# davidea97/Fisher-Nerf-customized

Hardware: AMD Instinct MI355X
Metric: candidate-views/sec (higher is better)
Workload: dtype f32

## Files before the change

### fisher-nerf-customized_amd/csrc/fisher_rast.hip

```cpp
#include <hip/hip_runtime.h>
#include <hip/hip_fp16.h>
#include <stdint.h>
#include <stdio.h>
#include <stdlib.h>
#include <string.h>
#include "fr_math.h"
#include "fr_sortnet.h"
#include "../../include/fisher_rast.h"
#include "fr_internal.h"

#define FR_THREADS 256
#define FR_G_MAX 32
#define FR_MAX_LDS_TILES 4096
#define FR_PART_MIN_DEFAULT 2048
#define FR_SORT_SMALL_KEYS 2048
#define FR_SORT_MID_KEYS 4096
#define FR_SORT_BIG_KEYS 16384
#define FR_VC_MAX 16
#define FR_BATCH 256
#define FR_BWD_BATCH 128

#include <vector>
#include <utility>
static thread_local char g_err[512] = "";
// ... 6 lines not shown
#define FR_AB_ONLY(x) x
static int fr_debug_mode();
static int fr_env_int(const char* name) { const char* e = getenv(name); return e ? atoi(e) : 0; }
#else
#define FR_AB_ONLY(x)
static constexpr int fr_debug_mode() { return 0; }
#endif
static bool g_prof_on = false;
static std::vector<std::pair<hipEvent_t, hipEvent_t>> g_prof_events;
int fr_fail(int code, const char* msg)
{
	snprintf(g_err, sizeof(g_err), "%s", msg);
	return code;
}
int fr_check_launch(const char* what)
{
	hipError_t e = hipGetLastError();
	if (e != hipSuccess)
	{
		snprintf(g_err, sizeof(g_err), "%s: %s", what, hipGetErrorString(e));
		return FR_ELAUNCH;
	}
	return FR_OK;
}

struct FrSplat { float x, y, cx, cy, cz, o, depth; uint32_t ext; };

struct FrVisEntry { uint32_t idx, depth_bits, xy0, xy1; };

struct FrParams {
	int P, V, W, H;
	uint32_t gx, gy;
	int T;
	int G;
	float tanfovx, tanfovy, focal_x, focal_y, mod;
	int D, M;
	const float* bg; const float* view; const float* proj; const float* campos;
	const float* w2c;
	const float* means3D; const float* colors; const float* shs; const float* opac;
	const float* scales; const float* rots;
	const float* cov3D;
	float* cov3D_out;
	int* radii;
	FrSplat* splat;
	float* rgb;
	uint8_t* clamped;
	uint32_t* tile_cnt; uint32_t* tile_off; uint32_t* tile_fill;
	uint64_t* keys; long long key_capacity;
	uint32_t* blk_base;
	uint32_t* big_list;
	uint32_t* view_work;
	uint32_t* part_list;
	uint32_t* view_perm;
	int* status;
	int* vis_count;
	int* num_rendered;
	struct FrVisEntry* vis_list;
	uint32_t* vis_n;
	int VC;
	uint32_t tile_cap;
	uint32_t small_max;
	const uint32_t* order;
	int legacy_sort;
	int prefiltered;
	int ablate;
};
#ifdef FR_ABLATE
#define FR_ABL(x) x
#else
#define FR_ABL(x)
#endif

__device__ __forceinline__ float wave_sum(float v)
{
#pragma unroll
	for (int o = 32; o > 0; o >>= 1) v += __shfl_xor(v, o, 64);
	return v;
}
__device__ __forceinline__ int wave_max_i(int v)
{
#pragma unroll
	for (int o = 32; o > 0; o >>= 1) { int t = __shfl_xor(v, o, 64); v = t > v ? t : v; }
	return v;
}

__device__ __forceinline__ bool fr_any(bool x) { return __builtin_amdgcn_ballot_w64(x) != 0ull; }
__device__ __forceinline__ bool fr_all(bool x) { return __builtin_amdgcn_ballot_w64(!x) == 0ull; }
__device__ __forceinline__ float fr_readlane_f(float x, int l) { return __int_as_float(__builtin_amdgcn_readlane(__float_as_int(x), l)); }
__device__ __forceinline__ float fr_bperm_f(float x, int l) { return __int_as_float(__builtin_amdgcn_ds_bpermute(l << 2, __float_as_int(x))); }

__device__ __forceinline__ float fr_exp_hw(float x) { return __builtin_amdgcn_exp2f(x * 1.44269504088896341f); }

__device__ __forceinline__ float fr_power_threshold(float opacity)
{
	return (opacity > 0.f) ? (-__logf(255.0f * opacity) - 0.01f) : INFINITY;
}

__device__ __forceinline__ uint32_t fr_alpha_extent(float cx, float cy, float cz, float opacity)
{
	const float thr = fr_power_threshold(opacity);
	float hx = INFINITY, hy = INFINITY;
	if (!(thr <= 0.f)) { hx = -1.f; hy = -1.f; }
	else
	{
		const float det = cx * cz - cy * cy;
		if (det > 0.f && cx > 0.f && cz > 0.f)
// ... 70 lines not shown
		if (p.prefiltered && p_view.z <= 0.001f) p.status[3] = 1;
		if (!(p_view.z <= 0.001f))
		{
			float c3[6];
#pragma unroll
			for (int k = 0; k < 6; k++) c3[k] = p.cov3D[6 * (size_t)i + k];
			s = fr_preprocess_one(po, c3, vm, pm, p.W, p.H, p.tanfovx, p.tanfovy, p.focal_x, p.focal_y, p.gx, p.gy);
		}
		p.radii[vP + i] = s.radius;
		if (s.radius > 0)
		{
			nvis++;
			float4* dst = (float4*)(p.splat + vP + i);
			dst[0] = make_float4(s.px, s.py, s.conx, s.cony);
			dst[1] = make_float4(s.conz, p.opac[i], s.depth, __uint_as_float(fr_alpha_extent(s.conx, s.cony, s.conz, p.opac[i])));
			if (p.colors == nullptr)
			{
				fr_f3 cp = { p.campos[0], p.campos[1], p.campos[2] };
				uint8_t cl[3];
				fr_f3 c = fr_sh_to_rgb(p.D, po, cp, p.shs + 3 * (size_t)i * p.M, cl);
				p.rgb[3 * (vP + i)] = c.x; p.rgb[3 * (vP + i) + 1] = c.y; p.rgb[3 * (vP + i) + 2] = c.z;
				p.clamped[3 * (vP + i)] = cl[0]; p.clamped[3 * (vP + i) + 1] = cl[1]; p.clamped[3 * (vP + i) + 2] = cl[2];
			}
			for (uint32_t y = s.rect.y0; y < s.rect.y1; y++)
				for (uint32_t x = s.rect.x0; x < s.rect.x1; x++)
				{
					if (lds_hist) atomicAdd(&hist[y * p.gx + x], 1u);
					else atomicAdd(&cnt[y * p.gx + x], 1u);
				}
		}
	}
	if (lds_hist)
	{
		__syncthreads();
		for (int t = tid; t < p.T; t += FR_THREADS)
		{
			uint32_t c = hist[t];
			if (c)
			{
				const uint32_t before = atomicAdd(&cnt[t], c);
				if (p.blk_base) p.blk_base[((size_t)v * gridDim.x + blockIdx.x) * p.T + t] = before;
			}
		}
	}
	if (p.vis_count)
	{
		int s = nvis;
#pragma unroll
		for (int o = 32; o > 0; o >>= 1) s += __shfl_xor(s, o, 64);
		if ((tid & 63) == 0 && s) atomicAdd(&p.vis_count[v], s);
	}
}

__device__ __forceinline__ void fr_deal_views(const uint32_t* __restrict__ work, uint32_t* __restrict__ perm, int V, int tid, int nthreads)
{
	__shared__ uint32_t s_work[1024];
	for (int v = tid; v < V; v += nthreads) s_work[v] = __hip_atomic_load(work + v, __ATOMIC_RELAXED, __HIP_MEMORY_SCOPE_AGENT);
	__syncthreads();
	for (int v = tid; v < V; v += nthreads)
	{
		const uint32_t w = s_work[v];
		int rank = 0;
		for (int u = 0; u < V; u++)
		{
			const uint32_t wu = s_work[u];
			rank += (wu > w || (wu == w && u < v)) ? 1 : 0;
		}
		const int r = rank >> 3, j = rank & 7;
		perm[r * 8 + ((r & 1) ? 7 - j : j)] = (uint32_t)v;
	}
}

__global__ __launch_bounds__(1024) void k_scan_tiles(const uint32_t* __restrict__ cnt, uint32_t* __restrict__ off,
                                                     uint32_t* __restrict__ fill, int N, int T, int V,
                                                     long long capacity, int* __restrict__ status,
                                                     int* __restrict__ num_rendered, uint32_t* __restrict__ big_list,
                                                     uint32_t* __restrict__ view_work, uint32_t* __restrict__ view_perm)
{
	__shared__ uint32_t wsum[16];
	__shared__ uint32_t chunk_total;
	const int tid = threadIdx.x, lane = tid & 63, wave = tid >> 6;
	uint32_t carry = 0, maxc = 0;
	constexpr int PER = 16;
	for (int sbase = 0; sbase < N; sbase += 1024 * PER)
	{
		const int i0 = sbase + tid * PER;
		uint32_t c[PER];
		uint32_t s = 0;
		const bool whole = i0 + PER <= N;
		if (whole)
		{
#pragma unroll
			for (int q = 0; q < PER / 4; q++)
			{
				const uint4 t4 = ((const uint4*)(cnt + i0))[q];
				c[4 * q] = t4.x; c[4 * q + 1] = t4.y; c[4 * q + 2] = t4.z; c[4 * q + 3] = t4.w;
			}
		}
		else
		{
#pragma unroll
			for (int q = 0; q < PER; q++) c[q] = (i0 + q < N) ? cnt[i0 + q] : 0u;
		}
#pragma unroll
		for (int q = 0; q < PER; q++)
		{
			s += c[q];
			maxc = c[q] > maxc ? c[q] : maxc;
			if (c[q] > (uint32_t)FR_SORT_SMALL_KEYS) big_list[16 + atomicAdd(&big_list[0], 1u)] = (uint32_t)(i0 + q);
		}
		uint32_t x = s;
#pragma unroll
		for (int d = 1; d < 64; d <<= 1)
		{
			uint32_t y = __shfl_up(x, d, 64);
			if (lane >= d) x += y;
		}
		if (lane == 63) wsum[wave] = x;
		__syncthreads();
		if (wave == 0)
		{
			uint32_t ws = lane < 16 ? wsum[lane] : 0u;
			uint32_t incl = ws;
// ... 862 lines not shown
#pragma unroll
			for (int b = 0; b < NB; b++)
			{
				const uint32_t e = e0 + b * FR_THREADS + tid;
				const uint32_t lo = ev[b] ? vend[ev[b] - 1] : 0u;
				const uint64_t key = ((uint64_t)en[b].x << 32) | ((blockIdx.x * cap + (e - lo)) << 4);
				const uint32_t r = en[b].y;
				const uint32_t x0 = r & 255u, s0 = (r >> 8) & 255u, x1 = x0 + ((r >> 16) & 255u), s1 = s0 + (r >> 24);
				const uint32_t* hb = hist + (size_t)ev[b] * p.T;
				uint32_t* cu = cursor + (size_t)ev[b] * p.T;
				if (x1 > x0 && s1 > s0)
				for (uint32_t y = s0 >> 2; y <= (s1 - 1u) >> 2; y++)
				{
					const uint32_t a = max(s0, 4u * y) - 4u * y, z = min(s1, 4u * y + 4u) - 4u * y;
					const uint64_t ky = key | (uint64_t)(((1u << z) - 1u) & ~((1u << a) - 1u));
					for (uint32_t x = x0; x < x1; x++)
					{
						const uint32_t t = y * p.gx + x;
						const uint32_t base = hb[t];
						const uint32_t k = atomicAdd(&cu[t], 1u);
						FR_ABL(if (p.ablate != 32 && p.ablate != 33))
						if (base != 0xffffffffu) p.keys[base + k] = ky;
					}
				}
			}
			if (more)
			{
#pragma unroll
				for (int b = 0; b < NB; b++) { en[b] = nx[b]; ev[b] = nxv[b]; }
			}
		}
	}
	else
	{
		for (int vv = 0; vv < nv; vv++)
		{
			const int v = v0 + vv;
			uint32_t* cnt = p.tile_cnt + (size_t)v * p.T;
			const uint32_t* h = hist + (size_t)vv * p.T;
			for (int t = tid; t < p.T; t += FR_THREADS)
			{
				const uint32_t c = h[t];
				if (c) p.blk_base[((size_t)v * nblk + blockIdx.x) * p.T + t] = atomicAdd(&cnt[t], c);
			}
		}
	}
	if (tid < nv)
	{
		const int v = v0 + tid;
		p.vis_n[(size_t)v * nblk + blockIdx.x] = s_n[tid];
		if (p.vis_count && s_n[tid]) atomicAdd(&p.vis_count[v], (int)s_n[tid]);
		if (p.num_rendered && s_ref[tid]) atomicAdd(&p.num_rendered[v], (int)s_ref[tid]);
	}
}
__global__ __launch_bounds__(FR_THREADS) void k_scatter_vis(FrParams p)
{
	extern __shared__ uint32_t fr_dyn_lds[];
	uint32_t* s_cnt = fr_dyn_lds;
	uint32_t* s_base = fr_dyn_lds + p.T;
	if (p.status[1]) return;
	const int tid = threadIdx.x;
	const int v = blockIdx.y;
	const uint32_t nblk = gridDim.x;
	const uint32_t n = p.vis_n[(size_t)v * nblk + blockIdx.x];
	if (n == 0) return;
	const uint32_t* off = p.tile_off + (size_t)v * p.T;
	const uint32_t* bb = p.blk_base + ((size_t)v * nblk + blockIdx.x) * p.T;
	for (int t = tid; t < p.T; t += FR_THREADS) { s_cnt[t] = 0; s_base[t] = off[t] + bb[t]; }
	__syncthreads();
	const uint4* list = (const uint4*)(p.vis_list + ((size_t)v * nblk + blockIdx.x) * (size_t)(FR_THREADS * p.G));
	constexpr int NB = 4;
	for (uint32_t e0 = 0; e0 < n; e0 += NB * FR_THREADS)
	{
		uint4 en[NB];
#pragma unroll
		for (int b = 0; b < NB; b++)
		{
			const uint32_t e = e0 + b * FR_THREADS + tid;
			en[b] = e < n ? list[e] : make_uint4(0u, 0u, 0u, 0u);
		}
#pragma unroll
		for (int b = 0; b < NB; b++)
		{
			const uint64_t key = ((uint64_t)en[b].y << 32) | en[b].x;
			const uint32_t x0 = en[b].z & 0xffffu, y0 = en[b].z >> 16, x1 = en[b].w & 0xffffu, y1 = en[b].w >> 16;
			for (uint32_t y = y0; y < y1; y++)
				for (uint32_t x = x0; x < x1; x++)
				{
					const uint32_t t = y * p.gx + x;
					p.keys[s_base[t] + atomicAdd(&s_cnt[t], 1u)] = key;
				}
		}
	}
}

__device__ __forceinline__ void fr_tile_of_block(const FrParams& p, uint32_t& tile, int& v, uint32_t first = 0u)
{
	const uint32_t L = blockIdx.x - first;
	if ((p.V & 7) == 0)
	{
		const uint32_t xcd = L & 7u, q = L >> 3;
		v = (int)((q / (uint32_t)p.T) * 8u + xcd);
		if (p.view_perm) v = (int)p.view_perm[v];
		tile = q % (uint32_t)p.T;
	}
	else
// ... 5190 lines not shown
	{
		if (hipDeviceGetAttribute(&cus, hipDeviceAttributeMultiprocessorCount, dev) != hipSuccess || cus <= 0) cus = 256;
		device = dev;
		(void)hipGetLastError();
	}
	return cus;
}

struct FrJoinGuard {
	hipStream_t s; FrSideStream* side[2] = { nullptr, nullptr }; int n = 0;
	explicit FrJoinGuard(hipStream_t caller) : s(caller) {}
	void forked(FrSideStream* ss) { side[n++] = ss; }
	int join()
	{
		int rc = FR_OK;
		for (int i = 0; i < n; i++)
		{
			if (hipEventRecord(side[i]->join, side[i]->stream) != hipSuccess || hipStreamWaitEvent(s, side[i]->join, 0) != hipSuccess)
				rc = fr_fail(FR_ELAUNCH, "side stream join failed");
		}
		n = 0;
		return rc;
	}
	~FrJoinGuard() { if (n) { char keep[sizeof(g_err)]; memcpy(keep, g_err, sizeof(keep)); (void)join(); memcpy(g_err, keep, sizeof(keep)); } }
};

enum class FrRecForm {
	Score,
	A,
	General,
	Pose,
	Render,
	Point,
};
struct FrScorerPlan {
	FrRecForm form = FrRecForm::Score;
	int columns;
	FrRecordArgs ra;
	bool skip_pack = false;
	bool view_identity = false;
};
template <int C> __global__ void k_pack_static(FrParams p, const float* __restrict__ H_inv, float* __restrict__ packed, float4* __restrict__ mt, float4* __restrict__ grp);
template <int C, bool LIST, bool FORM_A> __global__ void k_fisher_records(FrParams p, FrRecordArgs ra);

static int fr_bin_pipeline(FrParams& p, const fr_gaussians* g, hipStream_t s, const FrScorerPlan* plan = nullptr)
{
	int rc;
	const int P = p.P;
	{
		FrZeroer z;
		z.add(p.tile_cnt, (size_t)p.V * p.T * 4); z.add(p.status, 16); z.add(p.big_list, 64);
		if (p.part_list) z.add(p.part_list, 4);
		if (p.view_work) z.add(p.view_work, (size_t)p.V * 4);
		if (p.vis_count) z.add(p.vis_count, (size_t)p.V * 4);
		if (p.num_rendered && p.vis_list != nullptr && p.T <= FR_MAX_LDS_TILES) z.add(p.num_rendered, (size_t)p.V * 4);
		z.launch(s);
	}
	const bool multi = p.vis_list != nullptr && p.T <= FR_MAX_LDS_TILES;
	if (g->cov3D_precomp) p.cov3D = g->cov3D_precomp;
	else if (plan && multi) p.cov3D = nullptr;
	else
	{
		hipLaunchKernelGGL(k_cov3d, dim3((P + FR_THREADS - 1) / FR_THREADS), dim3(FR_THREADS), 0, s, P, g->scales, p.mod, g->rotations, p.cov3D_out);
		if ((rc = fr_check_launch("k_cov3d"))) return rc;
		p.cov3D = p.cov3D_out;
	}
	p.G = multi ? fr_pick_G_views(P) : fr_pick_G(P, p.V);
	p.VC = fr_pick_VC(p.T);
	const int per_block = FR_THREADS * p.G;
	dim3 gridP((P + per_block - 1) / per_block, p.V);
	const size_t hist_lds = p.T <= FR_MAX_LDS_TILES ? (size_t)p.T * 4 : 16;
	if (plan && !plan->skip_pack)
	{
		const float* shared_hinv = plan->ra.hinv_stride ? nullptr : plan->ra.H_inv;
		dim3 gp((P + FR_THREADS - 1) / FR_THREADS);
		if (plan->columns == 4) hipLaunchKernelGGL((k_pack_static<4>), gp, dim3(FR_THREADS), 0, s, p, shared_hinv, (float*)plan->ra.packed, (float4*)plan->ra.mt, (float4*)plan->ra.grp);
		else hipLaunchKernelGGL((k_pack_static<11>), gp, dim3(FR_THREADS), 0, s, p, shared_hinv, (float*)plan->ra.packed, (float4*)plan->ra.mt, (float4*)plan->ra.grp);
		if ((rc = fr_check_launch("k_pack_static"))) return rc;
	}
	FrJoinGuard joins(s);
	if (multi)
	{
		const bool once = plan && plan->ra.comp != nullptr && fr_debug_mode() != 20;
		if (!once) p.tile_cap = 0;
		const bool wanted_fixed = p.tile_cap != 0;
		if (once) p.VC = fr_plan_views_c(p.T, p.VC, p.tile_cap);
		if (once && wanted_fixed && !p.tile_cap) return fr_fail(FR_EINVAL, "fr_bin_pipeline: fixed key segments planned, but they do not fit the LDS");
		auto lds_c_of = [&](int vc) { return fr_lds_views_c(vc, p.T, p.tile_cap != 0); };
		dim3 gridV(gridP.x, (p.V + p.VC - 1) / p.VC);
		const size_t lds = ((size_t)p.VC * p.T + (size_t)FR_THREADS * p.VC + 12 * (size_t)p.VC + 2 * (size_t)p.VC * 8 * (size_t)p.G) * 4;
		FrRecordArgs ra = plan ? plan->ra : FrRecordArgs{ nullptr, 0, nullptr, nullptr, nullptr, nullptr, 0, nullptr, nullptr, 6 };
		const bool dk = p.tile_cap != 0;
		const size_t lds_c = lds_c_of(p.VC);
#define FR_VIEWS_C(...) hipLaunchKernelGGL((k_preprocess_views_c<__VA_ARGS__>), gridV, dim3(FR_THREADS), lds_c, s, p, ra)
		const bool c4 = plan && plan->columns == 4;
		if (once)
		{
			switch (plan->form)
			{
			case FrRecForm::Render:
				if (dk) FR_VIEWS_C(4, 4, true); else FR_VIEWS_C(4, 4, false);
				break;
			case FrRecForm::Pose:
				if (dk) FR_VIEWS_C(4, 3, true); else FR_VIEWS_C(4, 3, false);
				break;
			case FrRecForm::General:
				if (c4) { if (dk) FR_VIEWS_C(4, 2, true); else FR_VIEWS_C(4, 2, false); }
				else { if (dk) FR_VIEWS_C(11, 2, true); else FR_VIEWS_C(11, 2, false); }
				break;
			case FrRecForm::A:
				if (dk) FR_VIEWS_C(4, 1, true); else FR_VIEWS_C(4, 1, false);
				break;
			case FrRecForm::Point:
				if (c4) { if (dk) FR_VIEWS_C(4, 0, true, false, true); else FR_VIEWS_C(4, 0, false, false, true); }
				else { if (dk) FR_VIEWS_C(11, 0, true, false, true); else FR_VIEWS_C(11, 0, false, false, true); }
				break;
			case FrRecForm::Score:
				if (c4 && dk && plan->view_identity) FR_VIEWS_C(4, 0, true, true);
				else if (c4) { if (dk) FR_VIEWS_C(4, 0, true); else FR_VIEWS_C(4, 0, false); }
				else { if (dk) FR_VIEWS_C(11, 0, true); else FR_VIEWS_C(11, 0, false); }
				break;
			}
		}
#undef FR_VIEWS_C
		else if (!plan) hipLaunchKernelGGL((k_preprocess_views<0, false>), gridV, dim3(FR_THREADS), lds, s, p, ra);
#ifdef FR_AB
		else if (plan->form == FrRecForm::A) hipLaunchKernelGGL((k_preprocess_views<-4, true>), gridV, dim3(FR_THREADS), lds, s, p, ra);
		else if (c4) hipLaunchKernelGGL((k_preprocess_views<4, true>), gridV, dim3(FR_THREADS), lds, s, p, ra);
		else hipLaunchKernelGGL((k_preprocess_views<11, true>), gridV, dim3(FR_THREADS), lds, s, p, ra);
#else
		else return fr_fail(FR_EINVAL, "fr_bin_pipeline: a records plan of the multi-view front end needs compact records");
#endif
		if ((rc = fr_check_launch("k_preprocess_views"))) return rc;
	}
	else
	{
		p.tile_cap = 0;
		hipLaunchKernelGGL(k_preprocess, gridP, dim3(FR_THREADS), hist_lds, s, p);
		if ((rc = fr_check_launch("k_preprocess"))) return rc;
	}
	if (multi && p.tile_cap >= 2u * (uint32_t)FR_SORT_SMALL_KEYS + 128u && fr_debug_mode() != 32)
	{
		p.small_max = (uint32_t)FR_PART_MIN_DEFAULT;
		FR_AB_ONLY({ const int e = fr_env_int("FR_PART_MIN"); if (e >= 512 && e <= FR_SORT_SMALL_KEYS) p.small_max = (uint32_t)e; })
	}
	if (multi && p.tile_cap)
		hipLaunchKernelGGL(k_tile_lists, dim3((p.V * p.T + 4 * FR_THREADS - 1) / (4 * FR_THREADS)), dim3(FR_THREADS), 0, s, p.tile_cnt, p.tile_off, p.V * p.T, p.T,
		                   p.tile_cap, p.status, p.big_list, p.view_work, p.view_perm, p.ablate, p.small_max);
	else
	hipLaunchKernelGGL(k_scan_tiles, dim3(1), dim3(1024), 0, s, p.tile_cnt, p.tile_off, p.tile_fill, p.V * p.T, p.T, p.V,
	                   p.key_capacity, p.status, multi ? (int*)nullptr : p.num_rendered, p.big_list, p.view_work, p.view_perm);
	if ((rc = fr_check_launch("k_scan_tiles"))) return rc;
	if (multi && p.tile_cap) {  }
	else if (multi) hipLaunchKernelGGL(k_scatter_vis, gridP, dim3(FR_THREADS), 2 * hist_lds, s, p);
	else hipLaunchKernelGGL(k_scatter_keys, gridP, dim3(FR_THREADS), 2 * hist_lds, s, p);
	if ((rc = fr_check_launch("k_scatter_keys"))) return rc;
	if (plan && !multi)
	{
		FrSideStream& s2 = fr_side_stream(1);
		const bool forked2 = s2.ok && hipEventRecord(s2.fork, s) == hipSuccess && hipStreamWaitEvent(s2.stream, s2.fork, 0) == hipSuccess;
		hipStream_t rs = forked2 ? s2.stream : s;
		if (plan->form == FrRecForm::A) hipLaunchKernelGGL((k_fisher_records<4, false, true>), gridP, dim3(FR_THREADS), 0, rs, p, plan->ra);
		else if (plan->columns == 4) hipLaunchKernelGGL((k_fisher_records<4, false, false>), gridP, dim3(FR_THREADS), 0, rs, p, plan->ra);
		else hipLaunchKernelGGL((k_fisher_records<11, false, false>), gridP, dim3(FR_THREADS), 0, rs, p, plan->ra);
		if (forked2) joins.forked(&s2);
		if ((rc = fr_check_launch("k_fisher_records"))) return rc;
	}
	FrSideStream& side = fr_side_stream();
	const bool part_all = p.tile_cap >= 32768u && fr_debug_mode() != 32;
	const bool want_fork = fr_debug_mode() != 7 && (!multi || p.V >= 8) && !part_all;
	const bool forked = want_fork && side.ok && hipEventRecord(side.fork, s) == hipSuccess && hipStreamWaitEvent(side.stream, side.fork, 0) == hipSuccess;
	const int big_blocks = p.T * p.V < 256 ? p.T * p.V : 256;
	if (forked) joins.forked(&side);
	uint32_t part_max = 0;
	if (p.part_list && p.tile_cap >= 2u * (uint32_t)FR_SORT_SMALL_KEYS + 128u && fr_debug_mode() != 32)
	{
		part_max = p.tile_cap / 2u - 64u;
		if (part_max > 16320u) part_max = 16320u;
	}
	hipLaunchKernelGGL(k_sort_big_tiles, dim3(big_blocks), dim3(1024), 0, forked ? side.stream : s, p, part_max);
	if ((rc = fr_check_launch("k_sort_big_tiles"))) return rc;
	const int mid_blocks = p.T * p.V < 2048 ? p.T * p.V : 2048;
	if (part_max)
	{
		uint32_t split_blocks = (4u * (uint32_t)fr_cu_count()) & ~7u;
		if (split_blocks < 8u) split_blocks = 8u;
		if (split_blocks > (uint32_t)(p.T * p.V)) split_blocks = (uint32_t)(p.T * p.V);
		FR_AB_ONLY({ const int e = fr_env_int("FR_SPLIT_BLOCKS"); if (e >= 8 && e <= 8192) split_blocks = (uint32_t)e & ~7u; })
		hipLaunchKernelGGL(k_sort_split, dim3(split_blocks + (uint32_t)(p.T * p.V)), dim3(FR_THREADS), 0, s, p, part_max, split_blocks);
		if ((rc = fr_check_launch("k_sort_split"))) return rc;
		uint32_t part_blocks = 8u * (uint32_t)fr_cu_count();
		FR_AB_ONLY({ const int e = fr_env_int("FR_PART_BLOCKS"); if (e >= 1 && e <= 65536) part_blocks = (uint32_t)e; })
		hipLaunchKernelGGL(k_sort_parts, dim3(part_blocks), dim3(FR_THREADS), 0, s, p);
		if ((rc = fr_check_launch("k_sort_parts"))) return rc;
	}
	else
	{
		hipLaunchKernelGGL(k_sort_tiles, dim3(p.T * p.V), dim3(FR_THREADS), 0, s, p);
		if ((rc = fr_check_launch("k_sort_tiles"))) return rc;
// ... 375 lines not shown
	b.n_contrib = (const uint32_t*)((const char*)image_ws + L.n_contrib);
	b.power = 1;
	b.dL_dconic = dL_dconic; b.dL_dopacity = dL_dopacity;
	b.dL_dmean3D = dL_dmeans3D; b.dL_dcov3D = dL_dcov3D; b.dL_dscale = dL_dscales; b.dL_drot = dL_drotations;
	b.dL_dmean2D_b = nullptr;
	b.dL_dpix = dL_dout_color; b.colors = g->colors_precomp; b.dL_dmean2D = dL_dmeans2D; b.dL_dcolors = dL_dcolors;
	b.dL_dpix2 = dL_dout_features; b.colors2 = features; b.dL_dmean2D_2 = dL_dmeans2D_features; b.dL_dcolors2 = dL_dfeatures;
	b.only_flagged = nullptr; b.u_only = 0;
	const bool pair_walk = fr_debug_mode() == 18 || chunked;
	if (chunked)
	{
		if ((rc = fr_launch_chunked<6>(p, b, sq, scratch, nullptr, s))) return rc;
	}
	else
#ifdef FR_AB
	if (pair_walk)
	{
		hipLaunchKernelGGL((k_backward_lin_walk<true>), dim3(p.T), block, 0, s, p, b);
		if ((rc = fr_check_launch("k_backward_lin_walk<pair>"))) return rc;
	}
	else
#endif
	hipLaunchKernelGGL((k_backward_lin_tile<true>), dim3(p.T), block, 0, s, p, b, fallback);
	if ((rc = fr_check_launch("k_backward_lin_tile<pair>"))) return rc;
	for (int pass = 0; pass < 2 && !pair_walk; pass++)
	{
		b.dL_dpix = pass ? dL_dout_features : dL_dout_color;
		b.colors = pass ? features : g->colors_precomp;
		b.dL_dmean2D = pass ? dL_dmeans2D_features : dL_dmeans2D;
		b.dL_dcolors = pass ? dL_dfeatures : dL_dcolors;
		b.only_flagged = fallback; b.u_only = 1;
		if (sr) hipLaunchKernelGGL((k_backward_tile<true, false>), grid, block, 0, s, p, b);
		else hipLaunchKernelGGL((k_backward_tile<false, false>), grid, block, 0, s, p, b);
		if ((rc = fr_check_launch("k_backward_tile(flagged)"))) return rc;
	}
	b.dL_dmean2D = dL_dmeans2D; b.dL_dmean2D_b = dL_dmeans2D_features;
	b.dL_dcolors = dL_dcolors; b.colors = g->colors_precomp;
	dim3 gp((P + FR_THREADS - 1) / FR_THREADS);
	if (sr) hipLaunchKernelGGL((k_backward_finish<true, false>), gp, block, 0, s, p, b, (float*)nullptr);
	else hipLaunchKernelGGL((k_backward_finish<false, false>), gp, block, 0, s, p, b, (float*)nullptr);
	return fr_check_launch("k_backward_finish");
}

#ifdef FR_AB
static int fr_debug_mode()
{
	static const int mode = fr_env_int("FR_DEBUG_MODE");
	return mode;
}
#endif

#define FR_MAX_GROUPS 4
struct FrFisherLayout {
	size_t radii, vis_n, splat, recq, slot_idx, packed, mt, grp, big_list, part_list, view_work, view_perm, blk_base, cov3D, tile_cnt, tile_off, tile_fill, tile_scores, w2c_inv, status, keys, fallback, seg_T, seg_C, seg_X, seg_list, total;
	size_t PV;
};
static FrFisherLayout fr_fisher_layout(int64_t P, int64_t W, int64_t H, int64_t V, int64_t max_rendered, int columns)
{
	FrFisherLayout L;
	const int64_t T = ((W + 15) / 16) * ((H + 15) / 16);
	size_t o = 0;
	const size_t nblk_v = (size_t)fr_view_blocks(P);
	L.radii = o; o = fr_align(o + (size_t)V * nblk_v * (size_t)fr_view_block_slots(P) * sizeof(FrVisEntry));
	L.vis_n = o; o = fr_align(o + (size_t)V * nblk_v * 4);
	L.PV = nblk_v * (size_t)fr_view_block_slots(P);
	const size_t VPV = (size_t)V * (L.PV > (size_t)P ? L.PV : (size_t)P);
	L.splat = o; o = fr_align(o + VPV * sizeof(FrSplat));
	L.recq = o; o = fr_align(o + VPV * (columns == 11 ? 208 : 112));
	L.slot_idx = o; o = fr_align(o + VPV * 4);
	L.packed = o; o = fr_align(o + (size_t)P * 4 * (size_t)(columns == 11 ? 32 : 16));
	L.mt = o; o = fr_align(o + (size_t)P * 16);
	L.grp = o; o = fr_align(o + (size_t)((P + FR_THREADS - 1) / FR_THREADS) * 32);
	L.big_list = o; o = fr_align(o + (size_t)(V * T) * 4 + 64 * FR_MAX_GROUPS);
	L.view_work = o; o = fr_align(o + (size_t)V * 4);
	L.view_perm = o; o = fr_align(o + (size_t)V * 4);
	L.blk_base = o; o = fr_align(o + (size_t)V * (size_t)fr_preprocess_blocks(P, V) * (size_t)T * 4);
	L.cov3D = o; o = fr_align(o + (size_t)P * 24);
	L.tile_cnt = o; o = fr_align(o + (size_t)(V * T) * 4);
	L.tile_off = o; o = fr_align(o + (size_t)(V * T) * 4);
	L.tile_fill = o; o = fr_align(o + (size_t)(V * T) * 4);
	L.tile_scores = o; o = fr_align(o + (size_t)(V * T) * 4);
	L.w2c_inv = o; o = fr_align(o + (size_t)V * 64);
	L.status = o; o = fr_align(o + 64);
	const size_t R = (size_t)(max_rendered > 0 ? max_rendered : 1);
	L.keys = o; o = fr_align(o + R * 8);
	L.fallback = o; o = fr_align(o + (size_t)(V * T));
	const size_t seg_tiles = (size_t)(V * T <= FR_SEG_TILES ? V * T : 0);
	L.seg_T = o; o = fr_align(o + FR_SEG_PER_TILE * seg_tiles * FR_THREADS * 4);
	L.seg_C = o; o = fr_align(o + FR_SEG_PER_TILE * seg_tiles * FR_THREADS * 8);
	L.seg_X = o; o = fr_align(o + seg_tiles * FR_THREADS * 8);
	L.seg_list = o; o = fr_align(o + (FR_SEG_PER_TILE * seg_tiles + 1) * 4);
	L.part_list = o; o = fr_align(o + (size_t)(V * T) * FR_PART_MAXP * 8 + 64 * FR_MAX_GROUPS);
	L.total = o;
	return L;
}

static void fr_export_offsets(const FrFisherLayout& L, size_t o[8])
{
	o[0] = L.tile_cnt; o[1] = L.tile_off; o[2] = L.keys; o[3] = L.splat; o[4] = L.recq; o[5] = L.tile_scores; o[6] = L.status; o[7] = L.vis_n;
}

extern "C" int fr_fisher_workspace_layout(int32_t P, int32_t W, int32_t H, int32_t n_views, int64_t max_rendered, int32_t columns, size_t o[8])
{
	if (P < 0 || W <= 0 || H <= 0 || n_views <= 0 || max_rendered < 0 || (columns != 4 && columns != 11) || !o)
		return fr_fail(FR_EINVAL, "fr_fisher_workspace_layout: bad argument");
	const FrFisherLayout L = fr_fisher_layout(P, W, H, n_views, max_rendered, columns);
	fr_export_offsets(L, o);
	return FR_OK;
}

extern "C" int fr_fisher_part_list_offset(int32_t P, int32_t W, int32_t H, int32_t n_views, int64_t max_rendered, int32_t columns, size_t* offset)
{
	if (P < 0 || W <= 0 || H <= 0 || n_views <= 0 || max_rendered < 0 || (columns != 4 && columns != 11) || !offset)
		return fr_fail(FR_EINVAL, "fr_fisher_part_list_offset: bad argument");
	*offset = fr_fisher_layout(P, W, H, n_views, max_rendered, columns).part_list;
	return FR_OK;
}

extern "C" int fr_init(void)
{
	if (!fr_side_stream(0).ok || !fr_side_stream(1).ok || !fr_side_stream(2).ok) return fr_fail(FR_ELAUNCH, "fr_init: could not create the side streams");
	return FR_OK;
}

extern "C" size_t fr_fisher_workspace_bytes(int32_t P, int32_t W, int32_t H, int32_t n_views, int64_t max_rendered, int32_t columns)
{
	if (P < 0 || W <= 0 || H <= 0 || n_views <= 0 || max_rendered < 0 || (columns != 4 && columns != 11)) return 0;
	return fr_fisher_layout(P, W, H, n_views, max_rendered, columns).total;
}

namespace {
struct FrProfSpan {
	hipStream_t s; const bool on; hipEvent_t ev0 = nullptr, ev1 = nullptr;
	explicit FrProfSpan(hipStream_t stream) : s(stream), on(g_prof_on)
	{
		if (!on) return;
		(void)hipEventCreate(&ev0); (void)hipEventCreate(&ev1);
		(void)hipEventRecord(ev0, s);
	}
	~FrProfSpan()
	{
		if (!on) return;
		(void)hipEventRecord(ev1, s);
		g_prof_events.push_back(std::make_pair(ev0, ev1));
	}
// ... 69 lines not shown

enum { FR_CHK_CFG = 1, FR_CHK_MAX_RENDERED = 2, FR_CHK_TILES = 4, FR_CHK_SEGMENTS = 8, FR_CHK_ALL = 15 };
static int fr_check_views(const char* who, const char* cfg_what, unsigned checks, const fr_raster_cfg* cfg, const fr_fisher_cfg* fc,
                          int64_t max_rendered, const int32_t* status)
{
	static thread_local char buf[256];
	auto fail = [&](const char* what) { snprintf(buf, sizeof(buf), "%s: %s", who, what); return fr_fail(FR_EINVAL, buf); };
	if ((checks & FR_CHK_CFG) && (!fc || fc->n_views <= 0 || !fc->w2c || !status)) return fail(cfg_what);
	if ((checks & FR_CHK_SEGMENTS) && fc->tile_capacity < 0) return fail("negative tile_capacity");
	if ((checks & FR_CHK_MAX_RENDERED) && max_rendered < 0) return fail("negative max_rendered");
	const long long T = (long long)((cfg->image_width + 15) / 16) * ((cfg->image_height + 15) / 16);
	if ((checks & FR_CHK_TILES) && T > FR_MAX_LDS_TILES) return fail("images beyond 4096 tiles are not supported");
	if ((checks & FR_CHK_SEGMENTS) && fc->tile_capacity > 0)
	{
		const long long need = (long long)fc->n_views * T * (long long)fc->tile_capacity;
		if (need > max_rendered || need >= (1ll << 32)) return fail("n_views * tiles * tile_capacity exceeds max_rendered (or 2^32)");
	}
	return FR_OK;
}

static void fr_empty_map(const fr_fisher_cfg* fc, int32_t* status, hipStream_t s)
{
	const size_t V = (size_t)fc->n_views;
	if (fc->out_scores) (void)hipMemsetAsync(fc->out_scores, 0, V * 4, s);
	if (fc->out_vis_count) (void)hipMemsetAsync(fc->out_vis_count, 0, V * 4, s);
	if (fc->out_num_rendered) (void)hipMemsetAsync(fc->out_num_rendered, 0, V * 4, s);
	(void)hipMemsetAsync(status, 0, 16, s);
}

static int fr_carve_views(FrParams& p, const FrFisherLayout& L, char* ws, const fr_fisher_cfg* fc, int64_t max_rendered, hipStream_t s,
                          bool deal_views = true)
{
	const int V = p.V;
	p.prefiltered = 0;
	p.w2c = fc->w2c;
	if (fc->poses_are_c2w)
	{
		float* inv = (float*)(ws + L.w2c_inv);
		hipLaunchKernelGGL(k_invert_poses, dim3((V + 63) / 64), dim3(64), 0, s, V, fc->w2c, inv);
		if (int rc = fr_check_launch("k_invert_poses")) return rc;
		p.w2c = inv;
	}
	p.radii = (int*)(ws + L.radii);
	p.vis_list = (FrVisEntry*)p.radii;
	p.vis_n = (uint32_t*)(ws + L.vis_n);
	p.splat = (FrSplat*)(ws + L.splat);
	p.cov3D_out = (float*)(ws + L.cov3D);
	p.tile_cnt = (uint32_t*)(ws + L.tile_cnt);
	p.tile_off = (uint32_t*)(ws + L.tile_off);
	p.tile_fill = (uint32_t*)(ws + L.tile_fill);
	p.status = (int*)(ws + L.status);
	p.big_list = (uint32_t*)(ws + L.big_list);
	p.part_list = (uint32_t*)(ws + L.part_list);
	const bool deal = deal_views && (V & 7) == 0 && V <= 1024;
	p.view_work = deal ? (uint32_t*)(ws + L.view_work) : nullptr;
	p.view_perm = deal ? (uint32_t*)(ws + L.view_perm) : nullptr;
	p.blk_base = (uint32_t*)(ws + L.blk_base);
	p.keys = (uint64_t*)(ws + L.keys);
	p.key_capacity = max_rendered;
	p.vis_count = fc->out_vis_count;
	p.num_rendered = fc->out_num_rendered;
	p.order = fc->order;
	return FR_OK;
}

static void fr_plan_fixed_segments(FrParams& p, int tile_capacity)
{
	const bool slots_fit = fr_view_blocks(p.P) * fr_view_block_slots(p.P) < (1ll << 28);
	p.tile_cap = (tile_capacity > 0 && p.gx <= 255u && p.gy <= 63u && slots_fit) ? (uint32_t)tile_capacity : 0u;
	(void)fr_plan_views_c(p.T, fr_pick_VC(p.T), p.tile_cap);
}

static void fr_wire_records(FrScorerPlan& plan, FrFisherArgs& f, const FrFisherLayout& L, char* ws, int rstride, bool slot_table)
{
	plan.ra.H_inv = nullptr; plan.ra.hinv_stride = 0;
	plan.ra.packed = (const float*)(ws + L.packed); plan.ra.recq = (float4*)(ws + L.recq);
	plan.ra.mt = (const float4*)(ws + L.mt);
	plan.ra.grp = (const float4*)(ws + L.grp);
	plan.ra.early = 1;
	plan.ra.comp = (float4*)(ws + L.recq);
	plan.ra.stride = rstride;
	plan.ra.slot_idx = slot_table ? (uint32_t*)(ws + L.slot_idx) : nullptr;
	plan.ra.slot_acc = nullptr;
	f.recA = plan.ra.comp; f.ab_view = (long long)L.PV * rstride; f.ab_stride = rstride;
	f.recQ = plan.ra.comp + 2; f.q_view = (long long)L.PV * rstride; f.q_stride = rstride;
	f.slot_idx = plan.ra.slot_idx; f.slot_view = (long long)L.PV;
}

extern "C" int fr_fisher_views(const fr_raster_cfg* cfg, const fr_gaussians* g, const fr_fisher_cfg* fc,
                               void* workspace, size_t workspace_bytes, int64_t max_rendered,
                               int32_t* status, fr_stream_t stream)
{
	int rc = fr_validate(cfg, g, "fr_fisher_views");
	if (rc) return rc;
	if ((rc = fr_check_views("fr_fisher_views", "bad fisher cfg", FR_CHK_CFG, cfg, fc, max_rendered, status))) return rc;
	if (fc->columns != 4 && fc->columns != 11) return fr_fail(FR_EINVAL, "fr_fisher_views: columns must be 4 or 11");
	if (!g->colors_precomp) return fr_fail(FR_EINVAL, "fr_fisher_views: needs colors_precomp (the reference always passes rgb_colors)");
	if (fc->columns == 11 && !(g->scales && g->rotations)) return fr_fail(FR_EINVAL, "fr_fisher_views: columns=11 needs scales and rotations");
	if (fc->out_scores && !fc->H_inv) return fr_fail(FR_EINVAL, "fr_fisher_views: out_scores needs H_inv");
	if (!fc->H_inv && !fc->out_H) return fr_fail(FR_EINVAL, "fr_fisher_views: nothing to compute (no H_inv and no out_H)");
	if (fc->H_inv && !fc->out_scores) return fr_fail(FR_EINVAL, "fr_fisher_views: H_inv without out_scores");
	if (fc->dL_dpix_image && (fc->H_inv || !fc->out_H)) return fr_fail(FR_EINVAL, "fr_fisher_views: dL_dpix_image is for the out_H mode (no H_inv)");
	const int P = cfg->P, W = cfg->image_width, H = cfg->image_height, V = fc->n_views;
	hipStream_t s = (hipStream_t)stream;
	if (P == 0)
	{
// ... 18 lines not shown
	f.key_shift = 0;
	const bool v3 = fc->H_inv && !fc->out_H && !fc->dL_dpix_image && f.debug_mode != 1 && f.debug_mode != 9;
	const bool v3h = !fc->H_inv && fc->out_H && !fc->dL_dpix_image && fc->columns == 4 && f.debug_mode != 1 && f.debug_mode != 9;
	const bool multi_fe = p.vis_list != nullptr && p.T <= FR_MAX_LDS_TILES;
	const bool v3g = !fc->H_inv && fc->out_H && !v3h && multi_fe && !g->cov3D_precomp && f.debug_mode != 1 && f.debug_mode != 9 && f.debug_mode != 22 && f.debug_mode != 19;
	const bool compact = (v3 || v3h || v3g) && multi_fe && f.debug_mode != 19;
	if (compact && f.debug_mode != 8 && f.debug_mode != 24 && f.debug_mode != 20) fr_plan_fixed_segments(p, fc->tile_capacity);
	else p.tile_cap = 0;
	const int rstride = v3g ? (fc->columns == 11 ? 13 : 7) : ((v3 && p.tile_cap) ? 5 : 6);
	FrScorerPlan plan;
	plan.form = v3h ? FrRecForm::A : v3g ? FrRecForm::General : FrRecForm::Score;
	plan.columns = fc->columns;
	plan.view_identity = fc->view_is_identity != 0;
	fr_wire_records(plan, f, L, ws, rstride, v3h || v3g);
	plan.ra.H_inv = fc->H_inv; plan.ra.hinv_stride = fc->H_inv_view_stride;
	plan.ra.early = (g->cov3D_precomp || f.debug_mode == 15) ? 0 : 1;
	if (!compact)
	{
		plan.ra.comp = nullptr; plan.ra.slot_idx = nullptr;
		f.recA = (const float4*)p.splat; f.ab_view = (long long)P * 2; f.ab_stride = 2;
		f.recQ = plan.ra.recq; f.q_view = (long long)P * 4; f.q_stride = 4;
		f.slot_idx = nullptr; f.slot_view = 0;
		p.order = nullptr;
	}

	const bool multi = p.vis_list != nullptr && p.T <= FR_MAX_LDS_TILES;
	const int n_groups = (v3 && multi) ? fr_pick_groups(V) : 1;
	FrSideStream& tside = fr_side_stream(2);
	const bool use_side = n_groups > 1 && tside.ok;
	hipStream_t ts = use_side ? tside.stream : s;
	static thread_local hipEvent_t front_done[FR_MAX_GROUPS] = { nullptr, nullptr, nullptr, nullptr };
	const size_t nblk_v = (size_t)fr_view_blocks(P), cap_v = (size_t)fr_view_block_slots(P);
	const size_t rec_view = compact ? L.PV : (size_t)P;
	struct TileJoin {
		hipStream_t s; FrSideStream* side; bool on;
		~TileJoin() { if (on) { (void)hipEventRecord(side->join, side->stream); (void)hipStreamWaitEvent(s, side->join, 0); } }
	} tile_join{ s, &tside, false };
	for (int gi = 0; gi < n_groups; gi++)
	{
		const int per = n_groups > 1 ? ((V / n_groups + 7) / 8) * 8 : V;
		const int v0 = gi * per, Vg = (gi == n_groups - 1) ? V - v0 : per;
		if (Vg <= 0) break;
		FrParams pg = p;
		pg.V = Vg;
		pg.w2c = p.w2c + 16 * (size_t)v0;
		pg.radii = p.radii ? (int*)((char*)p.radii + (size_t)v0 * nblk_v * cap_v * sizeof(FrVisEntry)) : nullptr;
		pg.vis_list = p.vis_list + (size_t)v0 * nblk_v * cap_v;
		pg.vis_n = p.vis_n + (size_t)v0 * nblk_v;
		pg.splat = p.splat + (size_t)v0 * rec_view;
		pg.tile_cnt = p.tile_cnt + (size_t)v0 * p.T; pg.tile_off = p.tile_off + (size_t)v0 * p.T; pg.tile_fill = p.tile_fill + (size_t)v0 * p.T;
		pg.status = p.status + 4 * gi;
		pg.big_list = p.big_list + (size_t)v0 * p.T + 16 * gi;
		pg.part_list = p.part_list + (size_t)v0 * p.T * (2 * FR_PART_MAXP) + 16 * gi;
		if (p.view_perm && (Vg & 7) == 0) { pg.view_work = p.view_work + v0; pg.view_perm = p.view_perm + v0; }
		else { pg.view_work = nullptr; pg.view_perm = nullptr; }
		pg.blk_base = p.blk_base + (size_t)v0 * (size_t)fr_preprocess_blocks(P, V) * (size_t)p.T;
		pg.tile_cap = p.tile_cap;
		const long long k0 = (long long)((__int128)max_rendered * v0 / V), k1 = (long long)((__int128)max_rendered * (v0 + Vg) / V);
		pg.keys = p.keys + k0; pg.key_capacity = k1 - k0;
		pg.vis_count = p.vis_count ? p.vis_count + v0 : nullptr;
		pg.num_rendered = p.num_rendered ? p.num_rendered + v0 : nullptr;
		FrScorerPlan pl = plan;
		pl.skip_pack = gi > 0 || (fc->reuse_static != 0 && compact);
		if (pl.ra.hinv_stride) pl.ra.H_inv = plan.ra.H_inv + (size_t)v0 * plan.ra.hinv_stride;
		pl.ra.recq = plan.ra.recq + (size_t)v0 * rec_view * 4;
		if (pl.ra.comp) pl.ra.comp = plan.ra.comp + (size_t)v0 * L.PV * rstride;
		if (pl.ra.slot_idx) pl.ra.slot_idx = plan.ra.slot_idx + (size_t)v0 * L.PV;
		FrFisherArgs fg = f;
		fg.recA = f.recA + (size_t)v0 * f.ab_view; fg.recQ = f.recQ + (size_t)v0 * f.q_view;
		if (f.slot_idx) fg.slot_idx = f.slot_idx + (size_t)v0 * f.slot_view;
		fg.tile_scores = f.tile_scores + (size_t)v0 * p.T;
		if (f.H_inv && f.hinv_stride) fg.H_inv = f.H_inv + (size_t)v0 * f.hinv_stride;
		if (f.out_H && f.outH_stride) fg.out_H = f.out_H + (size_t)v0 * f.outH_stride;
		if (f.dL_img && f.dL_stride) fg.dL_img = f.dL_img + (size_t)v0 * f.dL_stride;

		if ((rc = fr_bin_pipeline(pg, g, s, (v3 || v3h || v3g) ? &pl : nullptr))) return rc;
		fg.key_shift = pg.tile_cap ? 4 : 0;
		if (use_side)
		{
			if (!front_done[gi] && hipEventCreateWithFlags(&front_done[gi], hipEventDisableTiming) != hipSuccess)
				return fr_fail(FR_ELAUNCH, "fr_fisher_views: hipEventCreate failed");
			if (hipEventRecord(front_done[gi], s) != hipSuccess || hipStreamWaitEvent(ts, front_done[gi], 0) != hipSuccess)
				return fr_fail(FR_ELAUNCH, "fr_fisher_views: fork to the tile stream failed");
			tile_join.on = true;
		}
		if (v3) fr_launch_fisher_v3(pg, fg, pl.ra.recq, ts);
		else if (v3h || v3g)
		{
			FrSegArgs sg;
			sg.snapT = (float*)(ws + L.seg_T); sg.snapC = (double*)(ws + L.seg_C); sg.X = (double*)(ws + L.seg_X);
			sg.list = (uint32_t*)(ws + L.seg_list);
			if (pg.V * pg.T > FR_SEG_TILES) sg.snapT = nullptr;
			if (v3h) fr_launch_fisher_v3h(pg, fg, pl.ra.recq, sg, ts);
			else fr_launch_fisher_v3g(pg, fg, fc->columns, fc->dL_dpix_image != nullptr, sg, ts);
		}
		else if (fc->columns == 4) fr_launch_fisher<4>(pg, fg, (float*)(ws + L.packed), (uint8_t*)(ws + L.fallback), ts);
		else fr_launch_fisher<11>(pg, fg, (float*)(ws + L.packed), (uint8_t*)(ws + L.fallback), ts);
		if ((rc = fr_check_launch("k_fisher_tile"))) return rc;
	}
	hipLaunchKernelGGL(k_reduce_scores, dim3(fc->out_scores ? V : 1), dim3(FR_THREADS), 0, ts, f.tile_scores, p.T, p.status, n_groups,
	                   fc->out_scores, status);
	if ((rc = fr_check_launch("k_reduce_scores"))) return rc;
	return FR_OK;
}

static size_t fr_pose_part_offset(int64_t P, int64_t W, int64_t H, int64_t V, int64_t max_rendered)
// ... 664 lines not shown
```

Before: 48810.

## Fuse tile-list construction into the last preprocess block per view group

Adds a per-view-group completion counter so that the last block of the multi-view preprocess kernel builds the fixed tile offsets, big-tile list, status counters and view work totals. The last group to finish then runs the view dealing, which removes the separate k_tile_lists launch. The small_max setup moves ahead of the preprocess launch so the fused path can use it. In exchange it adds a global atomic counter per block and serialises that epilogue work onto a single block per group. It also depends on correct zeroing and offsetting of the counter buffer for each view group.

```diff
diff --git a/fisher-nerf-customized_amd/csrc/fisher_rast.hip b/fisher-nerf-customized_amd/csrc/fisher_rast.hip
--- a/fisher-nerf-customized_amd/csrc/fisher_rast.hip
+++ b/fisher-nerf-customized_amd/csrc/fisher_rast.hip
@@ -82,6 +82,7 @@
 	uint32_t* view_work;
 	uint32_t* part_list;
 	uint32_t* view_perm;
+	uint32_t* fe_done;
 	int* status;
 	int* vis_count;
 	int* num_rendered;
@@ -258,9 +259,8 @@
 	}
 }
 
-__device__ __forceinline__ void fr_deal_views(const uint32_t* __restrict__ work, uint32_t* __restrict__ perm, int V, int tid, int nthreads)
-{
-	__shared__ uint32_t s_work[1024];
+__device__ __forceinline__ void fr_deal_views_in(uint32_t* s_work, const uint32_t* __restrict__ work, uint32_t* __restrict__ perm, int V, int tid, int nthreads)
+{
 	for (int v = tid; v < V; v += nthreads) s_work[v] = __hip_atomic_load(work + v, __ATOMIC_RELAXED, __HIP_MEMORY_SCOPE_AGENT);
 	__syncthreads();
 	for (int v = tid; v < V; v += nthreads)
@@ -275,6 +275,11 @@
 		const int r = rank >> 3, j = rank & 7;
 		perm[r * 8 + ((r & 1) ? 7 - j : j)] = (uint32_t)v;
 	}
+}
+__device__ __forceinline__ void fr_deal_views(const uint32_t* __restrict__ work, uint32_t* __restrict__ perm, int V, int tid, int nthreads)
+{
+	__shared__ uint32_t s_work[1024];
+	fr_deal_views_in(s_work, work, perm, V, tid, nthreads);
 }
 
 __global__ __launch_bounds__(1024) void k_scan_tiles(const uint32_t* __restrict__ cnt, uint32_t* __restrict__ off,
@@ -1243,6 +1248,61 @@
 		if (p.vis_count && s_n[tid]) atomicAdd(&p.vis_count[v], (int)s_n[tid]);
 		if (p.num_rendered && s_ref[tid]) atomicAdd(&p.num_rendered[v], (int)s_ref[tid]);
 	}
+	if constexpr (DK)
+	{
+		if (p.fe_done)
+		{
+			__shared__ uint32_t s_last;
+			if (tid == 0) s_last = __hip_atomic_fetch_add(p.fe_done + 16 + blockIdx.y, 1u, __ATOMIC_RELAXED, __HIP_MEMORY_SCOPE_AGENT) == nblk - 1u ? 1u : 0u;
+			__syncthreads();
+			if (s_last)
+			{
+				uint32_t* s_vw = park;
+				if (tid < FR_VC_MAX) s_vw[tid] = 0u;
+				__syncthreads();
+				uint32_t sum = 0, mx = 0;
+				const int nb = nv * p.T;
+				for (int b = tid; b < nb; b += FR_THREADS)
+				{
+					const int vv = b / p.T;
+					const uint32_t i = (uint32_t)(v0 + vv) * (uint32_t)p.T + (uint32_t)(b - vv * p.T);
+					const uint32_t c = __hip_atomic_load(p.tile_cnt + i, __ATOMIC_RELAXED, __HIP_MEMORY_SCOPE_AGENT);
+					p.tile_off[i] = i * p.tile_cap;
+					sum += c;
+					mx = c > mx ? c : mx;
+					if (c > p.small_max) p.big_list[16 + atomicAdd(&p.big_list[0], 1u)] = i;
+					if (p.view_work && c) atomicAdd(&s_vw[vv], c);
+				}
+#pragma unroll
+				for (int o = 32; o > 0; o >>= 1)
+				{
+					sum += (uint32_t)__shfl_xor((int)sum, o, 64);
+					const uint32_t t = (uint32_t)__shfl_xor((int)mx, o, 64);
+					mx = t > mx ? t : mx;
+				}
+				if (lane == 0)
+				{
+					if (sum) atomicAdd(&p.status[0], (int)sum);
+					if (mx) atomicMax(&p.status[2], (int)mx);
+					if (mx > p.tile_cap) { atomicOr(&p.status[1], 1); atomicOr(&p.status[3], 1); }
+					FR_ABL(if (p.ablate >= 30) atomicOr(&p.status[1], 1);)
+				}
+				if (p.view_perm)
+				{
+					__syncthreads();
+					if (tid < nv)
+					{
+						__hip_atomic_store(p.view_work + v0 + tid, s_vw[tid], __ATOMIC_RELAXED, __HIP_MEMORY_SCOPE_AGENT);
+						asm volatile("s_waitcnt vmcnt(0)" ::: "memory");
+					}
+					__syncthreads();
+					if (tid == 0) s_last = __hip_atomic_fetch_add(p.fe_done, 1u, __ATOMIC_RELAXED, __HIP_MEMORY_SCOPE_AGENT) == gridDim.y - 1u ? 1u : 0u;
+					__syncthreads();
+					if (s_last) fr_deal_views_in(s_vw, (const uint32_t*)p.view_work, p.view_perm, p.V, tid, FR_THREADS);
+				}
+			}
+		}
+	}
 }
 __global__ __launch_bounds__(FR_THREADS) void k_scatter_vis(FrParams p)
 {
@@ -6539,6 +6599,7 @@
 		z.add(p.tile_cnt, (size_t)p.V * p.T * 4); z.add(p.status, 16); z.add(p.big_list, 64);
 		if (p.part_list) z.add(p.part_list, 4);
 		if (p.view_work) z.add(p.view_work, (size_t)p.V * 4);
+		if (p.fe_done && p.tile_cap) z.add(p.fe_done, (size_t)(16 + p.V) * 4);
 		if (p.vis_count) z.add(p.vis_count, (size_t)p.V * 4);
 		if (p.num_rendered && p.vis_list != nullptr && p.T <= FR_MAX_LDS_TILES) z.add(p.num_rendered, (size_t)p.V * 4);
 		z.launch(s);
@@ -6573,6 +6634,12 @@
 		const bool wanted_fixed = p.tile_cap != 0;
 		if (once) p.VC = fr_plan_views_c(p.T, p.VC, p.tile_cap);
 		if (once && wanted_fixed && !p.tile_cap) return fr_fail(FR_EINVAL, "fr_bin_pipeline: fixed key segments planned, but they do not fit the LDS");
+		if (p.tile_cap >= 2u * (uint32_t)FR_SORT_SMALL_KEYS + 128u && fr_debug_mode() != 32)
+		{
+			p.small_max = (uint32_t)FR_PART_MIN_DEFAULT;
+			FR_AB_ONLY({ const int e = fr_env_int("FR_PART_MIN"); if (e >= 512 && e <= FR_SORT_SMALL_KEYS) p.small_max = (uint32_t)e; })
+		}
+		if (!p.tile_cap || fr_debug_mode() == 38) p.fe_done = nullptr;
 		auto lds_c_of = [&](int vc) { return fr_lds_views_c(vc, p.T, p.tile_cap != 0); };
 		dim3 gridV(gridP.x, (p.V + p.VC - 1) / p.VC);
 		const size_t lds = ((size_t)p.VC * p.T + (size_t)FR_THREADS * p.VC + 12 * (size_t)p.VC + 2 * (size_t)p.VC * 8 * (size_t)p.G) * 4;
@@ -6626,12 +6693,8 @@
 		hipLaunchKernelGGL(k_preprocess, gridP, dim3(FR_THREADS), hist_lds, s, p);
 		if ((rc = fr_check_launch("k_preprocess"))) return rc;
 	}
-	if (multi && p.tile_cap >= 2u * (uint32_t)FR_SORT_SMALL_KEYS + 128u && fr_debug_mode() != 32)
-	{
-		p.small_max = (uint32_t)FR_PART_MIN_DEFAULT;
-		FR_AB_ONLY({ const int e = fr_env_int("FR_PART_MIN"); if (e >= 512 && e <= FR_SORT_SMALL_KEYS) p.small_max = (uint32_t)e; })
-	}
-	if (multi && p.tile_cap)
+	if (multi && p.tile_cap && p.fe_done) {  }
+	else if (multi && p.tile_cap)
 		hipLaunchKernelGGL(k_tile_lists, dim3((p.V * p.T + 4 * FR_THREADS - 1) / (4 * FR_THREADS)), dim3(FR_THREADS), 0, s, p.tile_cnt, p.tile_off, p.V * p.T, p.T,
 		                   p.tile_cap, p.status, p.big_list, p.view_work, p.view_perm, p.ablate, p.small_max);
 	else
@@ -7113,7 +7176,7 @@
 
 #define FR_MAX_GROUPS 4
 struct FrFisherLayout {
-	size_t radii, vis_n, splat, recq, slot_idx, packed, mt, grp, big_list, part_list, view_work, view_perm, blk_base, cov3D, tile_cnt, tile_off, tile_fill, tile_scores, w2c_inv, status, keys, fallback, seg_T, seg_C, seg_X, seg_list, total;
+	size_t radii, vis_n, splat, recq, slot_idx, packed, mt, grp, big_list, part_list, view_work, view_perm, blk_base, cov3D, tile_cnt, tile_off, tile_fill, tile_scores, w2c_inv, status, keys, fallback, seg_T, seg_C, seg_X, seg_list, fe_done, total;
 	size_t PV;
 };
 static FrFisherLayout fr_fisher_layout(int64_t P, int64_t W, int64_t H, int64_t V, int64_t max_rendered, int columns)
@@ -7152,6 +7215,7 @@
 	L.seg_X = o; o = fr_align(o + seg_tiles * FR_THREADS * 8);
 	L.seg_list = o; o = fr_align(o + (FR_SEG_PER_TILE * seg_tiles + 1) * 4);
 	L.part_list = o; o = fr_align(o + (size_t)(V * T) * FR_PART_MAXP * 8 + 64 * FR_MAX_GROUPS);
+	L.fe_done = o; o = fr_align(o + (size_t)V * 4 + 64 * FR_MAX_GROUPS);
 	L.total = o;
 	return L;
 }
@@ -7327,6 +7391,7 @@
 	p.status = (int*)(ws + L.status);
 	p.big_list = (uint32_t*)(ws + L.big_list);
 	p.part_list = (uint32_t*)(ws + L.part_list);
+	p.fe_done = (uint32_t*)(ws + L.fe_done);
 	const bool deal = deal_views && (V & 7) == 0 && V <= 1024;
 	p.view_work = deal ? (uint32_t*)(ws + L.view_work) : nullptr;
 	p.view_perm = deal ? (uint32_t*)(ws + L.view_perm) : nullptr;
@@ -7451,6 +7516,7 @@
 		pg.status = p.status + 4 * gi;
 		pg.big_list = p.big_list + (size_t)v0 * p.T + 16 * gi;
 		pg.part_list = p.part_list + (size_t)v0 * p.T * (2 * FR_PART_MAXP) + 16 * gi;
+		pg.fe_done = p.fe_done + v0 + 16 * gi;
 		if (p.view_perm && (Vg & 7) == 0) { pg.view_work = p.view_work + v0; pg.view_perm = p.view_perm + v0; }
 		else { pg.view_work = nullptr; pg.view_perm = nullptr; }
 		pg.blk_base = p.blk_base + (size_t)v0 * (size_t)fr_preprocess_blocks(P, V) * (size_t)p.T;
```

Result: no change. 48770 (-0.1%).
